# jithinjosepkl/mpi-perf

Hardware: AMD Instinct MI355X
Metric: per-pair xGMI GB/s at 4 MB + 8 B latency us; all-pairs aggregate GB/s at 2/4/8 GPUs (higher is better)
Workload: dtype u8

## Files before the change

### mpi-perf_amd/csrc/mpx_internal.h

```cpp
#pragma once

#include <hip/hip_runtime.h>
#include <stdint.h>
#include <stddef.h>
#include "../../include/mpx.h"

typedef unsigned long long u64;

namespace mpx {

constexpr int kBlock = 256;
constexpr int kMaxPushWG = 256;
constexpr int kLLMaxBytes = 8192;
constexpr int kLLGranules = kLLMaxBytes / 4;
constexpr int kNbWindow = 256;
constexpr int kStageMaxBytes = 60 << 10;

enum Proto { kProtoLL = 0, kProtoBulk = 1, kProtoSdma = 2, kProtoRccl = 3, kProtoCopy = 4, kProtoCopySteps = 5,
             kProtoCopyPipe = 6, kProtoPull = 7, kProtoSdmaPull = 8 };

struct Mailbox {
    u64 flag[MPX_MAX_RANKS][kMaxPushWG];
    u64 ll[MPX_MAX_RANKS][kLLGranules];
    u64 credit[MPX_MAX_RANKS][kMaxPushWG];
// ... 42 lines not shown
constexpr u64 kGoCancel = 1ull << 63;

constexpr int kScratchWords = 16;
constexpr int kScrBar = 0, kScrAbort = 1, kScrFin = 2, kScrLanded = 3, kScrSeqBase = 4, kScrLink = 6, kScrGo = 8,
              kScrReady = 9;

inline int ring_slots(unsigned long long ring_bytes, long long len) {
    if (len <= 0) return kNbWindow;
    const unsigned long long s = 1 + ring_bytes / (unsigned long long)len;
    return s < (unsigned long long)kNbWindow ? (int)s : kNbWindow;
}
__host__ __device__ inline int ring_slot(int j, int iters, int slots) { return (iters - 1 - j) % slots; }

struct LatBlock {
    u64 count, calls, min_ticks, max_ticks, sum_ticks, max_iter, last_iters;
    u64 raw_cap;
    u64 raw_n;
    unsigned hist[MPX_LAT_BUCKETS];
    u64 raw[1];
};
inline size_t lat_block_bytes(int raw_cap) { return sizeof(LatBlock) + (size_t)raw_cap * sizeof(u64); }

struct XferArgs {
    const unsigned char* tx;
    unsigned char* rx;
    unsigned char* peer_rx;
    Mailbox* my_mb;
    Mailbox* peer_mb;
    Status* status;
    u64* csum;
    u64* gbar;
    u64 tx_seq0;
    u64 rx_seq0;
    u64 timeout_ticks;
    long long len;
    int iters;
    int mode;
    int group;
    int my_slot;
    int peer_slot;
    int nwg;
    int check;
    int ll_max;
    int stream;
    int nb_publish;
    int stage;
    unsigned char* ring;
    unsigned char* peer_ring;
    u64* cnt;
    int slots;
    int skip_push;
    u64 call;
    int lag_wg;
    u64 lag_ticks;
    const unsigned char* peer_tx;
    int pull;
    int no_pull_wait;
    u64 done_token;
    u64 go_token;
    u64 go_timeout_ticks;
    LatBlock* lat;
};

inline int ll_max_bytes(bool same_device) { return same_device ? 2048 : kLLMaxBytes; }

__host__ __device__ inline unsigned ll_tag(u64 seq) {
    return (unsigned)(seq & 0x7fffffffull) | 0x80000000u;
}

constexpr long long kMinPushChunk = 1024;
inline int bulk_nwg(long long len, bool same_device) {
    const long long per = same_device ? (16 << 10) : (32 << 10);
    long long n = (len + per - 1) / per;
    const long long cap = 128;
    if (n < 1) n = 1;
    if (n > cap) n = cap;
    return (int)n;
}

hipError_t launch_xfer(const XferArgs& a, int grid, hipStream_t s);
hipError_t launch_copy(void* dst, const void* src, size_t n, hipStream_t s, int* grid_out);
constexpr int kCopyStepsMaxGrid = 1024;
constexpr size_t kCopyStepsDefaultMax = (size_t)1 << 20;
constexpr size_t kCopyPipeDefaultMin = (size_t)512 << 10;
constexpr size_t kCopyPipeDefaultMax = (size_t)16 << 20;
hipError_t launch_copy_steps(void* dst, const void* src, size_t n, int iters, u64* bar, hipStream_t s,
                             int* grid_out, const int* shape = nullptr);
constexpr int kCopyPipeMaxGrid = 768;
hipError_t launch_copy_pipe(void* dst, const void* src, size_t n, int iters, u64* bar, hipStream_t s,
                            int* grid_out, int upl_force = 0, int hier_force = -1);
hipError_t launch_fill(void* p, size_t n, int pattern, u64 arg, hipStream_t s);
hipError_t launch_checksum(const void* p, size_t n, u64* out_dev, hipStream_t s);
hipError_t launch_signal(u64* flag, const u64* base, u64 value, hipStream_t s);
hipError_t launch_wait(const u64* flag, const u64* base, u64 value, Status* st, u64 timeout_ticks, hipStream_t s);
hipError_t launch_seqbase(u64* base, u64 tx, u64 rx, int add, hipStream_t s);
hipError_t launch_account(Status* st, const u64* csum, int j0, int count, long long n, hipStream_t s);

}
```

### mpi-perf_amd/csrc/mpx_kernels.hip

```cpp
#include "mpx_internal.h"

namespace mpx {

typedef unsigned int v4u __attribute__((ext_vector_type(4)));

constexpr u64 kGolden = 0x9E3779B97F4A7C15ull;
constexpr int kAuxSys = 17;
constexpr int kAuxSysNt = 19;
constexpr int kAuxSysVol = (int)0x80000011u;
constexpr int kLLUnits = kLLGranules / 2;
constexpr int kLLUnitsPerLane = kLLUnits / kBlock;
constexpr unsigned kRsrcWord3 = 0x00020000;

__device__ __forceinline__ u64 mix64(u64 z) {
    z = (z ^ (z >> 30)) * 0xbf58476d1ce4e5b9ull;
    z = (z ^ (z >> 27)) * 0x94d049bb133111ebull;
    return z ^ (z >> 31);
}
__device__ __forceinline__ u64 csum_term(u64 w, u64 k) { return mix64(w + (k + 1) * kGolden); }
__device__ __forceinline__ u64 fill_word(u64 key, u64 k) { return mix64((key ^ k) + kGolden); }

__device__ __forceinline__ u64 ld_sys(const u64* p) {
    return __hip_atomic_load(p, __ATOMIC_RELAXED, __HIP_MEMORY_SCOPE_SYSTEM);
}
// ... 144 lines not shown
        const unsigned g = blockIdx.x & 7;
        const u64 ng = (grid - g + 7) / 8;
        const u64 groups = grid < 8 ? grid : 8;
        for (int s = 0; s + 1 < iters; ++s) {
            wg_barrier_nofence();
            if (threadIdx.x == kPipeCopyWaves * 64) {
                s_stop = 0;
                u64 want;
                const u64* poll;
                if (hier) {
                    const u64 old = __hip_atomic_fetch_add(bar + 16 * (1 + g), 1ull, __ATOMIC_RELAXED,
                                                           __HIP_MEMORY_SCOPE_AGENT);
                    if (old + 1 == ng * (u64)(s + 1)) {
                        const u64 t = __hip_atomic_fetch_add(bar, 1ull, __ATOMIC_RELAXED, __HIP_MEMORY_SCOPE_AGENT);
                        if (t + 1 == groups * (u64)(s + 1))
                            for (u64 k = 0; k < groups; ++k)
                                __hip_atomic_store(bar + 16 * (9 + k), (u64)(s + 1), __ATOMIC_RELAXED,
                                                   __HIP_MEMORY_SCOPE_AGENT);
                    }
                    want = (u64)(s + 1);
                    poll = bar + 16 * (9 + g);
                } else {
                    __hip_atomic_fetch_add(bar, 1ull, __ATOMIC_RELAXED, __HIP_MEMORY_SCOPE_AGENT);
                    want = (u64)grid * (u64)(s + 1);
                    poll = bar;
                }
                const u64 t0 = now_ticks();
                u64 spins = 0;
                while (__hip_atomic_load(poll, __ATOMIC_RELAXED, __HIP_MEMORY_SCOPE_AGENT) < want) {
                    if ((++spins & 255) == 0 && now_ticks() - t0 > 100000000ull) {
                        __hip_atomic_store(&bar[1], 1ull, __ATOMIC_RELAXED, __HIP_MEMORY_SCOPE_AGENT);
                        s_stop = 1;
                        break;
                    }
                    __builtin_amdgcn_s_sleep(1);
                }
            }
            wg_barrier_nofence();
            if (s_stop) return;
        }
        return;
    }
    const unsigned stride16 = gridDim.x * (kPipeCopyWaves * 64) * 16u;
    const unsigned first16 = (blockIdx.x * (kPipeCopyWaves * 64) + threadIdx.x) * 16u;
    const unsigned body = (unsigned)(n16 * 16);
    const __amdgpu_buffer_rsrc_t rs = rsrc(src, body), rd = rsrc(dst, body);
    const unsigned tb = __builtin_amdgcn_readfirstlane((blockIdx.x == 0 && threadIdx.x < 64) ? tail : 0u);
    const __amdgpu_buffer_rsrc_t ts = rsrc(reinterpret_cast<const unsigned char*>(src) + body, tb);
    const __amdgpu_buffer_rsrc_t td = rsrc(reinterpret_cast<unsigned char*>(dst) + body, tb);
    v4u a[UPL], b[UPL];
    unsigned char ta, tb8;
    auto load = [&](v4u (&r)[UPL], unsigned char& t) {
        asm volatile("" ::: "memory");
#pragma unroll
        for (int u = 0; u < UPL; ++u)
            r[u] = __builtin_amdgcn_raw_buffer_load_b128(rs, first16 + u * stride16, 0, kAuxNt);
        t = __builtin_amdgcn_raw_buffer_load_b8(ts, threadIdx.x, 0, 0);
    };
    auto store = [&](v4u (&r)[UPL], unsigned char t) {
#pragma unroll
        for (int u = 0; u < UPL; ++u)
            __builtin_amdgcn_raw_buffer_store_b128(r[u], rd, first16 + u * stride16, 0, kAuxNt);
        __builtin_amdgcn_raw_buffer_store_b8(t, td, threadIdx.x, 0, 0);
    };
    auto grid_barrier = [&]() -> bool {
        wg_barrier_nofence();
        wg_barrier_nofence();
        return !s_stop;
    };
    load(a, ta);
    for (int s = 0;;) {
        if (s + 1 == iters) { store(a, ta); break; }
        load(b, tb8);
        store(a, ta);
        if (!grid_barrier()) break;
        if (++s + 1 == iters) { store(b, tb8); break; }
        load(a, ta);
        store(b, tb8);
        if (!grid_barrier()) break;
        ++s;
    }
}

__global__ __launch_bounds__(kBlock) void k_fill(unsigned char* p, size_t n, int pattern, u64 arg) {
    const size_t nw = n / 8;
    const size_t stride = (size_t)gridDim.x * kBlock;
    u64* p64 = reinterpret_cast<u64*>(p);
    const u64 bytew = (arg & 0xff) * 0x0101010101010101ull;
    for (size_t k = (size_t)blockIdx.x * kBlock + threadIdx.x; k < nw; k += stride)
        p64[k] = pattern == MPX_FILL_BYTE ? bytew : fill_word(arg, k);
    const unsigned tail = (unsigned)(n & 7);
    if (blockIdx.x == 0 && threadIdx.x < tail) {
        const u64 w = pattern == MPX_FILL_BYTE ? bytew : fill_word(arg, nw);
        p[nw * 8 + threadIdx.x] = (unsigned char)(w >> (8 * threadIdx.x));
    }
}

__device__ __forceinline__ u64 tail_word(const unsigned char* p, size_t off, size_t n) {
    u64 w = 0;
    for (size_t b = 0; off + b < n && b < 8; ++b) w |= (u64)p[off + b] << (8 * b);
    return w;
}

__global__ __launch_bounds__(kBlock) void k_checksum(const unsigned char* p, size_t n, u64* out) {
    __shared__ u64 lds4[4];
    const size_t n16 = n / 16;
    const size_t stride = (size_t)gridDim.x * kBlock;
    const v4u* p16 = reinterpret_cast<const v4u*>(p);
    u64 acc = 0;
    for (size_t v = (size_t)blockIdx.x * kBlock + threadIdx.x; v < n16; v += stride) {
        const v4u x = p16[v];
        acc += csum_term(((u64)x.y << 32) | x.x, 2 * v);
        acc += csum_term(((u64)x.w << 32) | x.z, 2 * v + 1);
    }
    if (blockIdx.x == 0 && threadIdx.x < 2) {
        const size_t off = n16 * 16 + 8 * threadIdx.x;
        if (off < n) acc += csum_term(tail_word(p, off, n), off / 8);
    }
    const u64 s = block_sum(acc, lds4);
    if (threadIdx.x == 0 && s) atomicAdd(out, s);
}

__device__ __forceinline__ u64 rel(const u64* base, u64 v) { return base ? ld_sys(base) + v : v; }

__global__ void k_signal(u64* flag, const u64* base, u64 v) {
    if (threadIdx.x == 0) st_sys(flag, rel(base, v));
}

__global__ void k_wait(const u64* flag, const u64* base, u64 v, Status* st, u64 timeout_ticks) {
    if (threadIdx.x != 0) return;
    if (__hip_atomic_load(&st->err, __ATOMIC_RELAXED, __HIP_MEMORY_SCOPE_SYSTEM)) return;
    const u64 want = rel(base, v);
    const u64 t0 = now_ticks();
    u64 spins = 0, seen;
    while ((seen = ld_sys(flag)) < want) {
        if ((++spins & 255) == 0 && now_ticks() - t0 > timeout_ticks) {
            st->seen = seen;
            st->want = want;
            __hip_atomic_store(&st->err, 1u, __ATOMIC_RELAXED, __HIP_MEMORY_SCOPE_SYSTEM);
            return;
        }
        __builtin_amdgcn_s_sleep(1);
    }
}

__global__ void k_seqbase(u64* base, u64 tx, u64 rx, int add) {
    if (threadIdx.x != 0) return;
    st_sys(base, add ? ld_sys(base) + tx : tx);
    st_sys(base + 1, add ? ld_sys(base + 1) + rx : rx);
}

enum { kTsEntry = 0, kTsPosted = 1, kTsFirst = 2, kTsLoop = 3 };

template <int MODE>
struct Loop {
    const XferArgs& a;
    int* s_abort;
    u64* lds4;
    v4u* s_tx;
    u64 pre[kLLUnitsPerLane];
    u64* s_seen = nullptr;
    mutable bool staged = false;
    mutable u64 ts[4] = {0, 0, 0, 0};
    mutable u64 rdone = 0, rdig = 0;

    __device__ void preload_ll(long long n) {
// ... 939 lines not shown
    }
    hipLaunchKernelGGL(k, dim3(grid), dim3(kBlock), (unsigned)a.stage, s, a);
    return hipGetLastError();
}

hipError_t launch_copy(void* dst, const void* src, size_t n, hipStream_t s, int* grid_out) {
    const size_t n16 = n / 16;
    const unsigned tail = (unsigned)(n & 15);
    size_t grid = (n16 + (size_t)kBlock - 1) / (size_t)kBlock;
    if (grid < 1) grid = 1;
    if (grid > ((size_t)1 << 31) - 1) return hipErrorInvalidValue;
    if (grid_out) *grid_out = (int)grid;
    (void)hipGetLastError();
    hipLaunchKernelGGL((k_copy<1, true, true, false>), dim3((unsigned)grid), dim3(kBlock), 0, s,
                       reinterpret_cast<const v4u*>(src), reinterpret_cast<v4u*>(dst), n16, tail);
    return hipGetLastError();
}

hipError_t launch_copy_steps(void* dst, const void* src, size_t n, int iters, u64* bar, hipStream_t s,
                             int* grid_out, const int* shape) {
    int cap = 64, xcd = 0, drain = 0, threads = 1024, upl = 1, one_xcd = 0;
    if (n > ((size_t)16 << 10) && n <= ((size_t)512 << 10)) {
        one_xcd = 1;
        threads = n <= ((size_t)128 << 10) ? 512 : 1024;
    } else if (n > ((size_t)1 << 20)) {
        threads = kBlock;
        upl = 8;
    }
    if (shape) {
        cap = shape[0]; xcd = shape[1]; drain = shape[2]; upl = shape[3]; threads = shape[4]; one_xcd = shape[5];
    }
    if (threads != 512 && threads != 1024) threads = kBlock;
    int max_grid = kCopyStepsMaxGrid * kBlock / threads;
    if (one_xcd) {
        max_grid /= 8;
        xcd = 0;
    }
    if (cap < 1 || cap > max_grid) cap = max_grid;
    if (upl < 1) upl = 1;
    const size_t n16 = n / 16;
    size_t grid = (n16 + (size_t)threads * upl - 1) / ((size_t)threads * upl);
    if (grid > (size_t)cap) grid = (size_t)cap;
    if (grid < 1) grid = 1;
    if (grid_out) *grid_out = (int)grid;
    (void)hipGetLastError();
    void (*k)(const v4u*, v4u*, size_t, unsigned, int, u64*, int, int) =
        threads == 1024 ? (xcd ? k_copy_steps<1024, true> : k_copy_steps<1024, false>)
        : threads == 512 ? (xcd ? k_copy_steps<512, true> : k_copy_steps<512, false>)
                         : (xcd ? k_copy_steps<kBlock, true> : k_copy_steps<kBlock, false>);
    hipLaunchKernelGGL(k, dim3((unsigned)(one_xcd ? grid * 8 : grid)), dim3((unsigned)threads), 0, s,
                       reinterpret_cast<const v4u*>(src), reinterpret_cast<v4u*>(dst), n16, (unsigned)(n & 15), iters,
                       bar, drain, one_xcd);
    return hipGetLastError();
}

hipError_t launch_copy_pipe(void* dst, const void* src, size_t n, int iters, u64* bar, hipStream_t s,
                            int* grid_out, int upl_force, int hier_force) {
    const size_t n16 = n / 16;
    const size_t lanes = (size_t)kPipeCopyWaves * 64;
    auto cap_of = [](int u) -> size_t { return u >= 16 ? 256 : u >= 8 ? 512 : (size_t)kCopyPipeMaxGrid; };
    const bool big = n > ((size_t)1 << 20);
    int upl = big ? 4 : 8;
    while (big && upl < 16 && (n16 + lanes * upl - 1) / (lanes * upl) > 256) upl *= 2;
    if (upl_force > 0) upl = upl_force;
    upl = upl <= 1 ? 1 : upl <= 2 ? 2 : upl <= 4 ? 4 : upl <= 8 ? 8 : 16;
    size_t grid = (n16 + lanes * upl - 1) / (lanes * upl);
    while (grid > cap_of(upl) && upl < 16) {
        upl *= 2;
        grid = (n16 + lanes * upl - 1) / (lanes * upl);
    }
    if (grid > cap_of(upl) || n >= ((size_t)1 << 32)) return hipErrorInvalidValue;
    if (grid < 1) grid = 1;
    if (grid_out) *grid_out = (int)grid;
    void (*k)(const v4u*, v4u*, size_t, unsigned, int, u64*, int) =
        upl <= 1 ? k_copy_pipe<1> : upl <= 2 ? k_copy_pipe<2> : upl <= 4 ? k_copy_pipe<4>
        : upl <= 8 ? k_copy_pipe<8> : k_copy_pipe<16>;
    const int hier = hier_force >= 0 ? (hier_force != 0) : (big ? 1 : 0);
    (void)hipGetLastError();
    hipLaunchKernelGGL(k, dim3((unsigned)grid), dim3(kPipeThreads), 0, s, reinterpret_cast<const v4u*>(src),
                       reinterpret_cast<v4u*>(dst), n16, (unsigned)(n & 15), iters, bar, hier);
    return hipGetLastError();
}

hipError_t launch_fill(void* p, size_t n, int pattern, u64 arg, hipStream_t s) {
    size_t grid = (n / 8 + kBlock - 1) / kBlock;
    if (grid > 4096) grid = 4096;
    if (grid < 1) grid = 1;
    (void)hipGetLastError();
    hipLaunchKernelGGL(k_fill, dim3((unsigned)grid), dim3(kBlock), 0, s, reinterpret_cast<unsigned char*>(p), n,
                       pattern, arg);
    return hipGetLastError();
}

hipError_t launch_checksum(const void* p, size_t n, u64* out_dev, hipStream_t s) {
    size_t grid = (n / 16 + kBlock - 1) / kBlock;
    if (grid > 2048) grid = 2048;
    if (grid < 1) grid = 1;
    (void)hipGetLastError();
    hipLaunchKernelGGL(k_checksum, dim3((unsigned)grid), dim3(kBlock), 0, s, reinterpret_cast<const unsigned char*>(p),
                       n, out_dev);
    return hipGetLastError();
}

hipError_t launch_signal(u64* flag, const u64* base, u64 value, hipStream_t s) {
    (void)hipGetLastError();
    hipLaunchKernelGGL(k_signal, dim3(1), dim3(64), 0, s, flag, base, value);
    return hipGetLastError();
}

hipError_t launch_wait(const u64* flag, const u64* base, u64 value, Status* st, u64 timeout_ticks, hipStream_t s) {
    (void)hipGetLastError();
    hipLaunchKernelGGL(k_wait, dim3(1), dim3(64), 0, s, flag, base, value, st, timeout_ticks);
    return hipGetLastError();
}

hipError_t launch_seqbase(u64* base, u64 tx, u64 rx, int add, hipStream_t s) {
    (void)hipGetLastError();
    hipLaunchKernelGGL(k_seqbase, dim3(1), dim3(64), 0, s, base, tx, rx, add);
    return hipGetLastError();
}

hipError_t launch_account(Status* st, const u64* csum, int j0, int count, long long n, hipStream_t s) {
    const u64 z = (u64)n;
    u64 m = (z ^ (z >> 30)) * 0xbf58476d1ce4e5b9ull;
    m = (m ^ (m >> 27)) * 0x94d049bb133111ebull;
    m ^= m >> 31;
    (void)hipGetLastError();
    hipLaunchKernelGGL(k_account, dim3(1), dim3(kBlock), 0, s, st, csum, j0, count, m);
    return hipGetLastError();
}

}
```

### mpi-perf_amd/csrc/mpx_runtime.hip

```cpp
#include "mpx_internal.h"

#include <hsa/hsa.h>
#include <hsa/hsa_ext_amd.h>
#include <rccl/rccl.h>

#include <atomic>
#include <condition_variable>
#include <map>
#include <mutex>
#include <string>
#include <tuple>
#include <type_traits>
#include <vector>

#include <dlfcn.h>
#include <stdarg.h>
#include <stdio.h>
#include <string.h>
#include <time.h>
#include <unistd.h>

using namespace mpx;

namespace {
// ... 262 lines not shown
    HIPCK(hipGetDeviceCount(&n));
    if (dev < 0 || dev >= n) return fail(MPX_ERR_INVALID, "device %d out of range [0,%d)", dev, n);
    return MPX_OK;
}

int alloc_mailbox(Rank& rk) {
    const unsigned flags[2] = {hipDeviceMallocUncached, hipDeviceMallocFinegrained};
    for (int k = 0; k <= 1; ++k) {
        void* p = nullptr;
        if (hipExtMallocWithFlags(&p, sizeof(Mailbox), flags[k]) != hipSuccess) {
            (void)hipGetLastError();
            continue;
        }
        hipIpcMemHandle_t h;
        const hipError_t e = hipIpcGetMemHandle(&h, p);
        if (getenv("MPX_DEBUG"))
            fprintf(stderr, "[mpx] mailbox kind %d alloc ok, ipc handle: %s\n", k, hipGetErrorString(e));
        (void)hipGetLastError();
        if (e != hipSuccess) {
            (void)hipFree(p);
            continue;
        }
        rk.mb = static_cast<Mailbox*>(p);
        rk.mb_kind = k;
        return MPX_OK;
    }
    void* p = nullptr;
    HIPCK(hipMalloc(&p, sizeof(Mailbox)));
    if (getenv("MPX_DEBUG")) fprintf(stderr, "[mpx] mailbox kind 2 (coarse hipMalloc)\n");
    rk.mb = static_cast<Mailbox*>(p);
    rk.mb_kind = kMbCoarse;
    return MPX_OK;
}

int ensure_csum(Rank& rk, int iters) {
    if ((size_t)iters <= rk.csum_cap) return MPX_OK;
    if (rk.csum) rk.retired.push_back(rk.csum);
    rk.csum = rk.cnt = nullptr;
    size_t cap = 1024;
    while (cap < (size_t)iters) cap *= 2;
    HIPCK(hipMalloc(&rk.csum, 2 * cap * sizeof(u64)));
    rk.cnt = rk.csum + cap;
    rk.csum_cap = cap;
    return MPX_OK;
}

uint64_t ring_bytes_for(size_t len) {
    static const uint64_t cap = [] {
        const char* v = getenv("MPX_CHECK_RING_BYTES");
        return v ? (uint64_t)strtoull(v, nullptr, 0) : (uint64_t)64 << 20;
    }();
    if (len == 0) return 0;
    const uint64_t want = (uint64_t)(kNbWindow - 1) * len;
    const uint64_t slots = (want < cap ? want : cap) / len;
    return slots * len;
}

int ensure_ring(Rank& rk) {
    if (!rk.local || rk.ring) return MPX_OK;
    const uint64_t bytes = ring_bytes_for(rk.len);
    if (!bytes) return MPX_OK;
    DeviceGuard g(rk.dev);
    HIPCK(g.err);
    void* p = nullptr;
    const hipError_t e = hipMalloc(&p, bytes);
    if (e == hipErrorOutOfMemory)
        return fail(MPX_ERR_NOMEM, "check ring of %llu B on device %d", (unsigned long long)bytes, rk.dev);
    HIPCK(e);
    rk.ring = static_cast<unsigned char*>(p);
    rk.ring_bytes = bytes;
    return MPX_OK;
}

int link_slots(const Rank& a, const Rank& b, long long len) {
    const int sa = ring_slots(a.ring_bytes, len), sb = ring_slots(b.ring_bytes, len);
    return sa < sb ? sa : sb;
}

unsigned char* slot_ptr(const Rank& rk, int j, int iters, int slots, long long len) {
    const int s = ring_slot(j, iters, slots);
    return s == 0 ? rk.rx : rk.ring + (long long)(s - 1) * len;
}

enum CopyForm { kCopyAuto = 0, kCopyLaunch, kCopySteps, kCopyPipe };
struct CopyChoice {
    int form = kCopyAuto;
    bool shaped = false;
    int shape[6] = {0, 0, 0, 0, 0, 0};
    int upl = 0, hier = -1;
};
CopyChoice copy_choice() {
    CopyChoice c;
    const char* v = getenv("MPX_COPY");
    if (!v || !*v) return c;
    if (!strncmp(v, "launch", 6)) {
        c.form = kCopyLaunch;
    } else if (!strncmp(v, "steps", 5)) {
        c.form = kCopySteps;
        int* x = c.shape;
        const int k = sscanf(v + 5, ":%d:%d:%d:%d:%d:%d", &x[0], &x[1], &x[2], &x[3], &x[4], &x[5]);
        c.shaped = k >= 5;
    } else if (!strncmp(v, "pipe", 4)) {
        c.form = kCopyPipe;
        (void)sscanf(v + 4, ":%d:%d", &c.upl, &c.hier);
    }
    return c;
}

u64 nb_waited(int iters) {
    return (u64)iters - (u64)(iters / kNbWindow);
}

struct TestKnobs {
    int skip_push = 0;
    int lag_rank = -1, lag_wg = 0;
    long long lag_us = 0;
    bool no_posted = false, no_pull_wait = false;
    int fail_launch = -1;
    bool fail_copy = false;
};
bool test_gate() {
    static const bool gate = getenv("MPX_TEST") != nullptr;
    return gate;
}
TestKnobs test_knobs() {
    TestKnobs k;
    if (!test_gate()) return k;
    const char* v = getenv("MPX_TEST");
    if (!v) return k;
    std::string all(v);
    size_t pos = 0;
    while (pos <= all.size()) {
        size_t end = all.find(',', pos);
        if (end == std::string::npos) end = all.size();
        const std::string item = all.substr(pos, end - pos);
        if (!item.compare(0, 10, "skip_push=")) k.skip_push = atoi(item.c_str() + 10);
        else if (!item.compare(0, 7, "lag_wg=")) {
            if (sscanf(item.c_str() + 7, "%d:%d:%lld", &k.lag_rank, &k.lag_wg, &k.lag_us) != 3) k.lag_rank = -1;
        } else if (item == "no_posted") k.no_posted = true;
        else if (item == "no_pull_wait") k.no_pull_wait = true;
        else if (!item.compare(0, 12, "fail_launch=")) k.fail_launch = atoi(item.c_str() + 12);
        else if (item == "fail_copy") k.fail_copy = true;
        pos = end + 1;
    }
    return k;
}

struct StreamPool {
    std::mutex mu;
    std::map<int, std::vector<hipStream_t>> idle;
    std::vector<std::pair<int, hipStream_t>> all;
    int live_contexts = 0;
};
StreamPool& pool() {
    static StreamPool* p = new StreamPool;
    return *p;
}

void fence_cb(void* p) { static_cast<std::atomic<int>*>(p)->fetch_add(1, std::memory_order_release); }

bool on_events_thread(hsa_signal_value_t, void* arg) {
    static_cast<std::atomic<int>*>(arg)->store(1, std::memory_order_release);
    return false;
}

bool event_thread_barrier() {
    static hsa_signal_t sig = [] {
        hsa_signal_t s{0};
        if (hsa_signal_create(0, 0, nullptr, &s) != HSA_STATUS_SUCCESS) s.handle = 0;
        return s;
    }();
    if (!sig.handle) return false;
    const double t_end = now_s() + 10.0;
    for (int k = 0; k < 2; ++k) {
        std::atomic<int>* done = new std::atomic<int>(0);
        if (hsa_amd_signal_async_handler(sig, HSA_SIGNAL_CONDITION_EQ, 0, on_events_thread, done) != HSA_STATUS_SUCCESS) {
            delete done;
            return false;
        }
        while (!done->load(std::memory_order_acquire) && now_s() < t_end) usleep(20);
        if (!done->load(std::memory_order_acquire)) return false;
        delete done;
    }
    return true;
}

bool callback_fence(const std::vector<std::pair<int, hipStream_t>>& ss) {
// ... 925 lines not shown
}

int mpx_free(mpx_ctx* ctx, void* ptr) {
    if (!ctx) return fail(MPX_ERR_INVALID, "ctx is NULL");
    if (!ptr) return MPX_OK;
    AllocRec rec;
    {
        std::lock_guard<std::mutex> lk(ctx->mu);
        auto it = ctx->allocs.find(reinterpret_cast<uintptr_t>(ptr));
        if (it == ctx->allocs.end()) return fail(MPX_ERR_INVALID, "%p was not allocated by mpx_alloc", ptr);
        rec = it->second;
        ctx->allocs.erase(it);
    }
    DeviceGuard g(rec.dev);
    HIPCK(hipFree(ptr));
    return MPX_OK;
}

int mpx_fill(mpx_ctx* ctx, int dev, void* ptr, size_t n, int pattern, uint64_t arg) {
    if (!ctx || (!ptr && n)) return fail(MPX_ERR_INVALID, "NULL argument");
    if (pattern != MPX_FILL_BYTE && pattern != MPX_FILL_SPLITMIX) return fail(MPX_ERR_INVALID, "pattern %d", pattern);
    if (n && (reinterpret_cast<uintptr_t>(ptr) & 7)) return fail(MPX_ERR_INVALID, "fill buffer must be 8-byte aligned");
    TRY(check_dev(dev));
    if (!n) return MPX_OK;
    hipStream_t s;
    TRY(util_stream(ctx, dev, &s));
    std::lock_guard<std::mutex> ul(ctx->util_mu);
    DeviceGuard g(dev);
    HIPCK(launch_fill(ptr, n, pattern, arg, s));
    HIPCK(hipStreamSynchronize(s));
    return MPX_OK;
}

int mpx_checksum(mpx_ctx* ctx, int dev, const void* ptr, size_t n, uint64_t* out) {
    if (!ctx || !out || (!ptr && n)) return fail(MPX_ERR_INVALID, "NULL argument");
    if (n && (reinterpret_cast<uintptr_t>(ptr) & 15))
        return fail(MPX_ERR_INVALID, "checksum buffer must be 16-byte aligned");
    TRY(check_dev(dev));
    hipStream_t s;
    TRY(util_stream(ctx, dev, &s));
    std::lock_guard<std::mutex> ul(ctx->util_mu);
    u64* tmp = ctx->dev_tmp[dev];
    DeviceGuard g(dev);
    u64 raw = 0;
    if (n) {
        HIPCK(hipMemsetAsync(tmp, 0, sizeof(u64), s));
        HIPCK(launch_checksum(ptr, n, tmp, s));
        HIPCK(hipMemcpyAsync(&raw, tmp, sizeof(u64), hipMemcpyDeviceToHost, s));
        HIPCK(hipStreamSynchronize(s));
    }
    *out = raw ^ mix64_host((u64)n);
    return MPX_OK;
}

int mpx_read(mpx_ctx* ctx, int dev, void* host_dst, const void* dev_src, size_t n) {
    if (!ctx || ((!host_dst || !dev_src) && n)) return fail(MPX_ERR_INVALID, "NULL argument");
    TRY(check_dev(dev));
    if (!n) return MPX_OK;
    hipStream_t s;
    TRY(util_stream(ctx, dev, &s));
    std::lock_guard<std::mutex> ul(ctx->util_mu);
    DeviceGuard g(dev);
    HIPCK(hipMemcpyAsync(host_dst, dev_src, n, hipMemcpyDeviceToHost, s));
    HIPCK(hipStreamSynchronize(s));
    return MPX_OK;
}

int mpx_copy(mpx_ctx* ctx, int dev, void* dst, const void* src, size_t n, int iters, mpx_timing* t) {
    if (!ctx || !t || ((!dst || !src) && n) || iters < 0) return fail(MPX_ERR_INVALID, "bad argument");
    if ((reinterpret_cast<uintptr_t>(dst) | reinterpret_cast<uintptr_t>(src)) & 15)
        return fail(MPX_ERR_INVALID, "copy buffers must be 16-byte aligned");
    TRY(check_dev(dev));
    memset(t, 0, sizeof *t);
    hipStream_t s;
    TRY(util_stream(ctx, dev, &s));
    std::lock_guard<std::mutex> ul(ctx->util_mu);
    DeviceGuard g(dev);
    Event e0, e1;
    HIPCK(e0.create());
    HIPCK(e1.create());
    int grid = 0;
    const CopyChoice cc = copy_choice();
    const bool multi = n && iters > 1;
    bool pipe = multi && (cc.form == kCopyPipe ||
                          (cc.form == kCopyAuto && n > kCopyPipeDefaultMin && n <= kCopyPipeDefaultMax));
    const bool steps = multi && !pipe && (cc.form == kCopySteps || (cc.form == kCopyAuto && n <= kCopyPipeDefaultMin));
    bool one = pipe || steps;
    u64* bar = ctx->dev_tmp[dev] + 16;
    float ms = 0;
    double t0 = 0;
    for (int attempt = 0; attempt < 2; ++attempt) {
        if (one) HIPCK(hipMemsetAsync(bar, 0, 17 * 16 * sizeof(u64), s));
        t0 = now_s();
        HIPCK(hipEventRecord(e0, s));
        if (test_knobs().fail_copy) return fail(MPX_ERR_HIP, "copy failed after its start event (MPX_TEST fail_copy)");
        if (one && pipe) {
            const hipError_t e = launch_copy_pipe(dst, src, n, iters, bar, s, &grid, cc.upl, cc.hier);
            if (e == hipErrorInvalidValue) {
                (void)hipGetLastError();
                one = pipe = false;
                continue;
            }
            HIPCK(e);
        } else if (one)
            HIPCK(launch_copy_steps(dst, src, n, iters, bar, s, &grid, cc.shaped ? cc.shape : nullptr));
        else
            for (int i = 0; i < iters && n; ++i) HIPCK(launch_copy(dst, src, n, s, &grid));
        HIPCK(hipEventRecord(e1, s));
        HIPCK(hipEventSynchronize(e1));
        HIPCK(hipEventElapsedTime(&ms, e0, e1));
        if (!one) break;
        u64 stop = 0;
        HIPCK(hipMemcpyAsync(&stop, bar + 1, sizeof stop, hipMemcpyDeviceToHost, s));
        HIPCK(hipStreamSynchronize(s));
        if (!stop) break;
        DBG("copy of %zu B: step barrier gave up, a launch per copy instead\n", n);
        one = false;
    }
    t->wall_s = now_s() - t0;
    t->device_s = ms * 1e-3;
    t->bytes = (uint64_t)n * (uint64_t)iters;
    t->launches = !n ? 0 : one ? 1 : iters;
    t->nwg = grid;
    t->protocol = !one ? kProtoCopy : pipe ? kProtoCopyPipe : kProtoCopySteps;
    return MPX_OK;
}

namespace {

int attach_resources(Rank& rk) {
    HIPCK(hipDeviceGetPCIBusId(rk.bus_id, sizeof rk.bus_id, rk.dev));
    TRY(alloc_mailbox(rk));
    TRY(create_rank_stream(rk.dev, &rk.stream));
    HIPCK(hipMemsetAsync(rk.mb, 0, sizeof(Mailbox), rk.stream));
    HIPCK(rk.ev0.create());
    HIPCK(rk.ev1.create());
    HIPCK(hipHostMalloc(reinterpret_cast<void**>(&rk.status), sizeof(Status), hipHostMallocCoherent | hipHostMallocMapped));
    memset(rk.status, 0, sizeof(Status));
    HIPCK(hipMalloc(&rk.scratch, kScratchWords * sizeof(u64)));
    HIPCK(hipMemsetAsync(rk.scratch, 0, kScratchWords * sizeof(u64), rk.stream));
    TRY(ensure_csum(rk, 1024));
    HIPCK(hipStreamSynchronize(rk.stream));
    return MPX_OK;
}

void release_rank(Rank& rk) {
    if (rk.stream) (void)hipStreamSynchronize(rk.stream);
    if (rk.mb) (void)hipFree(rk.mb);
    if (rk.ring) (void)hipFree(rk.ring);
    if (rk.scratch) (void)hipFree(rk.scratch);
    if (rk.csum) (void)hipFree(rk.csum);
    if (rk.lat) (void)hipFree(rk.lat);
    for (void* q : rk.retired) (void)hipFree(q);
    if (rk.status) (void)hipHostFree(rk.status);
    rk.ev0.reset();
    rk.ev1.reset();
    if (rk.stream) release_rank_stream(rk.dev, rk.stream);
    (void)hipGetLastError();
    rk = Rank{};
}

int enable_peer_access(mpx_ctx* ctx, int dev) {
    for (int i = 0; i < MPX_MAX_RANKS; ++i) {
        const Rank& o = ctx->r[i];
        if (!o.local || o.dev == dev) continue;
        int can = 0;
        HIPCK(hipDeviceCanAccessPeer(&can, dev, o.dev));
        if (!can) return fail(MPX_ERR_UNSUPPORTED, "GPU %d cannot access GPU %d (no xGMI/P2P path)", dev, o.dev);
        for (int dir = 0; dir < 2; ++dir) {
            const int a = dir ? o.dev : dev, b = dir ? dev : o.dev;
            DeviceGuard ga(a);
            const hipError_t e = hipDeviceEnablePeerAccess(b, 0);
            if (e != hipSuccess && e != hipErrorPeerAccessAlreadyEnabled) HIPCK(e);
            (void)hipGetLastError();
        }
    }
    return MPX_OK;
}

}

int mpx_rank_attach(mpx_ctx* ctx, int rank, int dev, void* tx, void* rx, size_t len) {
    if (!ctx) return fail(MPX_ERR_INVALID, "ctx is NULL");
    if (rank < 0 || rank >= ctx->nranks) return fail(MPX_ERR_INVALID, "rank %d not in [0,%d)", rank, ctx->nranks);
    if (!tx || !rx) return fail(MPX_ERR_INVALID, "NULL tx/rx");
    if (len > 0x7fffffffull) return fail(MPX_ERR_INVALID, "len %zu exceeds the reference's int buff_len", len);
    TRY(check_dev(dev));
    {
        std::lock_guard<std::mutex> lk(ctx->mu);
        if (ctx->r[rank].local || ctx->r[rank].imported) return fail(MPX_ERR_STATE, "rank %d already registered", rank);
        auto it = ctx->allocs.find(reinterpret_cast<uintptr_t>(rx));
        if (it == ctx->allocs.end() || it->second.dev != dev || it->second.bytes < len)
            return fail(MPX_ERR_INVALID, "rx must be an mpx_alloc base on device %d of >= %zu bytes", dev, len);
        auto jt = ctx->allocs.find(reinterpret_cast<uintptr_t>(tx));
// ... 545 lines not shown
```

Before: 3268.

## Add single-workgroup repeated-copy kernel for small copies using workgroup barriers

```diff
diff --git a/mpi-perf_amd/csrc/mpx_internal.h b/mpi-perf_amd/csrc/mpx_internal.h
--- a/mpi-perf_amd/csrc/mpx_internal.h
+++ b/mpi-perf_amd/csrc/mpx_internal.h
@@ -148,6 +148,7 @@
 hipError_t launch_copy(void* dst, const void* src, size_t n, hipStream_t s, int* grid_out);
 constexpr int kCopyStepsMaxGrid = 1024;
 constexpr size_t kCopyStepsDefaultMax = (size_t)1 << 20;
+constexpr size_t kCopyOneMax = (size_t)32 << 10;
 constexpr size_t kCopyPipeDefaultMin = (size_t)512 << 10;
 constexpr size_t kCopyPipeDefaultMax = (size_t)16 << 20;
 hipError_t launch_copy_steps(void* dst, const void* src, size_t n, int iters, u64* bar, hipStream_t s,
@@ -155,6 +156,8 @@
 constexpr int kCopyPipeMaxGrid = 768;
 hipError_t launch_copy_pipe(void* dst, const void* src, size_t n, int iters, u64* bar, hipStream_t s,
                             int* grid_out, int upl_force = 0, int hier_force = -1);
+hipError_t launch_copy_one(void* dst, const void* src, size_t n, int iters, hipStream_t s, int* grid_out,
+                           int upl_force = 0);
 hipError_t launch_fill(void* p, size_t n, int pattern, u64 arg, hipStream_t s);
 hipError_t launch_checksum(const void* p, size_t n, u64* out_dev, hipStream_t s);
 hipError_t launch_signal(u64* flag, const u64* base, u64 value, hipStream_t s);
diff --git a/mpi-perf_amd/csrc/mpx_kernels.hip b/mpi-perf_amd/csrc/mpx_kernels.hip
--- a/mpi-perf_amd/csrc/mpx_kernels.hip
+++ b/mpi-perf_amd/csrc/mpx_kernels.hip
@@ -250,6 +250,72 @@
     }
 }
 
+constexpr int kOneThreads = 1024;
+
+template <int UPL, bool BODY, bool TAIL>
+__device__ __forceinline__ void one_wave_copies(__amdgpu_buffer_rsrc_t rs, __amdgpu_buffer_rsrc_t rd,
+                                                __amdgpu_buffer_rsrc_t ts, __amdgpu_buffer_rsrc_t td, int iters) {
+    constexpr unsigned stride16 = kOneThreads * 16u;
+    const unsigned first16 = threadIdx.x * 16u;
+    v4u a[UPL], b[UPL];
+    unsigned char ta = 0, tb8 = 0;
+    auto load = [&](v4u (&r)[UPL], unsigned char& t) {
+        asm volatile("" ::: "memory");
+        if constexpr (BODY) {
+#pragma unroll
+            for (int u = 0; u < UPL; ++u)
+                r[u] = __builtin_amdgcn_raw_buffer_load_b128(rs, first16 + u * stride16, 0, kAuxNt);
+        }
+        if constexpr (TAIL) t = __builtin_amdgcn_raw_buffer_load_b8(ts, threadIdx.x, 0, 0);
+    };
+    auto store = [&](v4u (&r)[UPL], unsigned char t) {
+        if constexpr (BODY) {
+#pragma unroll
+            for (int u = 0; u < UPL; ++u)
+                __builtin_amdgcn_raw_buffer_store_b128(r[u], rd, first16 + u * stride16, 0, kAuxNt);
+        }
+        if constexpr (TAIL) __builtin_amdgcn_raw_buffer_store_b8(t, td, threadIdx.x, 0, 0);
+    };
+    auto trip = [&]() {
+        load(b, tb8);
+        store(a, ta);
+        wg_barrier_nofence();
+        load(a, ta);
+        store(b, tb8);
+        wg_barrier_nofence();
+    };
+    load(a, ta);
+    int left = iters - 1;
+    if (left >= 2) {
+        trip();
+        for (left -= 2; left >= 2; left -= 2) trip();
+    }
+    if (left == 1) {
+        load(b, tb8);
+        store(a, ta);
+        wg_barrier_nofence();
+        store(b, tb8);
+    } else {
+        store(a, ta);
+    }
+}
+
+template <int UPL>
+__global__ __launch_bounds__(kOneThreads) void k_copy_one(const v4u* src, v4u* dst, size_t n16, unsigned tail,
+                                                        int iters) {
+    const unsigned body = (unsigned)(n16 * 16);
+    const __amdgpu_buffer_rsrc_t rs = rsrc(src, body), rd = rsrc(dst, body);
+    const __amdgpu_buffer_rsrc_t ts = rsrc(reinterpret_cast<const unsigned char*>(src) + body, tail);
+    const __amdgpu_buffer_rsrc_t td = rsrc(reinterpret_cast<unsigned char*>(dst) + body, tail);
+    const unsigned wave_first = __builtin_amdgcn_readfirstlane(threadIdx.x & ~63u);
+    const bool has_body = wave_first < n16;
+    const bool has_tail = wave_first == 0 && tail;
+    if (has_body && has_tail) one_wave_copies<UPL, true, true>(rs, rd, ts, td, iters);
+    else if (has_body) one_wave_copies<UPL, true, false>(rs, rd, ts, td, iters);
+    else if (has_tail) one_wave_copies<UPL, false, true>(rs, rd, ts, td, iters);
+    else for (int s = 0; s + 1 < iters; ++s) wg_barrier_nofence();
+}
+
 __global__ __launch_bounds__(kBlock) void k_fill(unsigned char* p, size_t n, int pattern, u64 arg) {
     const size_t nw = n / 8;
     const size_t stride = (size_t)gridDim.x * kBlock;
@@ -1355,6 +1421,22 @@
     return hipGetLastError();
 }
 
+hipError_t launch_copy_one(void* dst, const void* src, size_t n, int iters, hipStream_t s, int* grid_out,
+                           int upl_force) {
+    const size_t n16 = n / 16;
+    int upl = 1;
+    while (upl < 8 && n > (size_t)kOneThreads * 16 * upl) upl *= 2;
+    if (upl_force > 0) upl = upl_force <= 1 ? 1 : upl_force <= 2 ? 2 : upl_force <= 4 ? 4 : 8;
+    if (n > (size_t)kOneThreads * 16 * upl || iters < 1) return hipErrorInvalidValue;
+    if (grid_out) *grid_out = 1;
+    void (*k)(const v4u*, v4u*, size_t, unsigned, int) =
+        upl == 1 ? k_copy_one<1> : upl == 2 ? k_copy_one<2> : upl == 4 ? k_copy_one<4> : k_copy_one<8>;
+    (void)hipGetLastError();
+    hipLaunchKernelGGL(k, dim3(1), dim3(kOneThreads), 0, s, reinterpret_cast<const v4u*>(src),
+                       reinterpret_cast<v4u*>(dst), n16, (unsigned)(n & 15), iters);
+    return hipGetLastError();
+}
+
 hipError_t launch_fill(void* p, size_t n, int pattern, u64 arg, hipStream_t s) {
     size_t grid = (n / 8 + kBlock - 1) / kBlock;
     if (grid > 4096) grid = 4096;
diff --git a/mpi-perf_amd/csrc/mpx_runtime.hip b/mpi-perf_amd/csrc/mpx_runtime.hip
--- a/mpi-perf_amd/csrc/mpx_runtime.hip
+++ b/mpi-perf_amd/csrc/mpx_runtime.hip
@@ -368,7 +368,7 @@
     return s == 0 ? rk.rx : rk.ring + (long long)(s - 1) * len;
 }
 
-enum CopyForm { kCopyAuto = 0, kCopyLaunch, kCopySteps, kCopyPipe };
+enum CopyForm { kCopyAuto = 0, kCopyLaunch, kCopySteps, kCopyPipe, kCopyOne };
 struct CopyChoice {
     int form = kCopyAuto;
     bool shaped = false;
@@ -389,6 +389,9 @@
     } else if (!strncmp(v, "pipe", 4)) {
         c.form = kCopyPipe;
         (void)sscanf(v + 4, ":%d:%d", &c.upl, &c.hier);
+    } else if (!strncmp(v, "one", 3)) {
+        c.form = kCopyOne;
+        (void)sscanf(v + 3, ":%d", &c.upl);
     }
     return c;
 }
@@ -1480,23 +1483,26 @@
     int grid = 0;
     const CopyChoice cc = copy_choice();
     const bool multi = n && iters > 1;
+    bool wg1 = multi && (cc.form == kCopyOne || (cc.form == kCopyAuto && n <= kCopyOneMax));
     bool pipe = multi && (cc.form == kCopyPipe ||
                           (cc.form == kCopyAuto && n > kCopyPipeDefaultMin && n <= kCopyPipeDefaultMax));
-    const bool steps = multi && !pipe && (cc.form == kCopySteps || (cc.form == kCopyAuto && n <= kCopyPipeDefaultMin));
-    bool one = pipe || steps;
+    const bool steps = multi && !pipe && !wg1 &&
+                       (cc.form == kCopySteps || (cc.form == kCopyAuto && n <= kCopyPipeDefaultMin));
+    bool one = pipe || steps || wg1;
     u64* bar = ctx->dev_tmp[dev] + 16;
     float ms = 0;
     double t0 = 0;
     for (int attempt = 0; attempt < 2; ++attempt) {
-        if (one) HIPCK(hipMemsetAsync(bar, 0, 17 * 16 * sizeof(u64), s));
+        if (one && !wg1) HIPCK(hipMemsetAsync(bar, 0, 17 * 16 * sizeof(u64), s));
         t0 = now_s();
         HIPCK(hipEventRecord(e0, s));
         if (test_knobs().fail_copy) return fail(MPX_ERR_HIP, "copy failed after its start event (MPX_TEST fail_copy)");
-        if (one && pipe) {
-            const hipError_t e = launch_copy_pipe(dst, src, n, iters, bar, s, &grid, cc.upl, cc.hier);
+        if (one && (pipe || wg1)) {
+            const hipError_t e = wg1 ? launch_copy_one(dst, src, n, iters, s, &grid, cc.upl)
+                                     : launch_copy_pipe(dst, src, n, iters, bar, s, &grid, cc.upl, cc.hier);
             if (e == hipErrorInvalidValue) {
                 (void)hipGetLastError();
-                one = pipe = false;
+                one = pipe = wg1 = false;
                 continue;
             }
             HIPCK(e);
@@ -1507,7 +1513,7 @@
         HIPCK(hipEventRecord(e1, s));
         HIPCK(hipEventSynchronize(e1));
         HIPCK(hipEventElapsedTime(&ms, e0, e1));
-        if (!one) break;
+        if (!one || wg1) break;
         u64 stop = 0;
         HIPCK(hipMemcpyAsync(&stop, bar + 1, sizeof stop, hipMemcpyDeviceToHost, s));
         HIPCK(hipStreamSynchronize(s));
```

New measurement: 3268, median of 2. No clear change (+0.0%).
